# JiuTongBro/MultiView_Inpaint

Hardware: AMD Instinct MI355X
Metric: Mpix/s fwd+bwd @1.5M Gauss 1080p (higher is better)
Workload: dtype f32; 1 GPU; rasterizer-with-depth fwd+bwd, one 1920x1080 view per GPU per step, N=1500000 Gaussians, sh_degree 3 (BASELINE.json configs[2] size, SURVEY.md §8d scene); gaussians=1500000, visible=1312313, num_rendered_D=14779663, tiles=8160, tile_list_max=2266, parallelism=views x1

## Files before the change

include/mvi_raster.h:

```cpp
#ifndef MVI_RASTER_H
#define MVI_RASTER_H

#include <stddef.h>
#include <stdint.h>

#ifdef __cplusplus
extern "C" {
#endif

#define MVI_OK 0
#define MVI_EINVAL (-1)
#define MVI_EHIP (-2)
#define MVI_ENOMEM (-3)

#define MVI_TILE 16

typedef struct mvi_raster_settings {
    int32_t image_height;
    int32_t image_width;
    float tanfovx;
    float tanfovy;
    float scale_modifier;
    int32_t sh_degree;
    int32_t prefiltered;
// ... 65 lines not shown
                             const float* colors_precomp, const float* scales, const float* rotations,
                             const float* cov3D_precomp, const int32_t* radii, const void* geom,
                             const float* grad_rows_scratch, float* dL_dmeans3D, float* dL_dmeans2D, float* dL_dopacity,
                             float* dL_dshs, float* dL_dcolors, float* dL_dscales, float* dL_drotations, float* dL_dcov3D,
                             void* stream);

int mvi_raster_backward_geom_range(const mvi_raster_settings* s, int32_t P, int32_t M, int32_t first, int32_t count,
                                   const float* means3D, const float* shs, const float* colors_precomp, const float* scales,
                                   const float* rotations, const float* cov3D_precomp, const int32_t* radii, const void* geom,
                                   const float* grad_rows_scratch, float* dL_dmeans3D, float* dL_dmeans2D, float* dL_dopacity,
                                   float* dL_dshs, float* dL_dcolors, float* dL_dscales, float* dL_drotations, float* dL_dcov3D,
                                   void* stream);

typedef struct mvi_raster_views {
    const float* depths;
    const float* means2D;
    const float* cov3D_a;
    const float* cov3D_b;
    const float* conic_opacity;
    const float* rgbd;
    const uint32_t* tiles_touched;
    const uint8_t* clamped;
    const void* tile_ids_sorted;
    const uint32_t* point_list;
    const uint32_t* ranges;
    const float* final_T;
    const uint32_t* n_contrib;
    int32_t tile_id_bytes;
    const uint8_t* grad_support;
} mvi_raster_views;
int mvi_raster_get_views(int32_t P, int64_t num_rendered, int32_t image_width, int32_t image_height,
                         const void* geom, const void* binning, const void* image,
                         mvi_raster_views* out);

#define MVI_RASTER_NSTAGES 8
int mvi_raster_timing_enable(int enable);
int mvi_raster_timing_enable_stages(uint32_t stage_mask);
int mvi_raster_timing_read(float* ms_sum_host, int32_t* calls_host);
const char* mvi_raster_stage_name(int stage);

int mvi_raster_color_mode(int deferred);
int mvi_raster_resolve_colors(const mvi_raster_settings* s, int32_t P, void* geom, size_t geom_bytes, void* stream);

int mvi_raster_binning_version(int version);
int mvi_raster_backward_mode(int dense);
int mvi_raster_dev_stamps(int pass, void* device_buffer);
int mvi_raster_dev_wave_sum9(const float* in, float* out, int n_waves, void* stream);

const char* mvi_raster_last_error(void);
const char* mvi_version(void);

#ifdef __cplusplus
}
#endif
#endif
```

multiview_inpaint_amd/_lib.py:

```python
import ctypes as C
import os
import re

_HERE = os.path.dirname(os.path.abspath(__file__))
LIB_PATH = os.environ.get("MVI_HIP_LIB") or os.path.join(_HERE, "csrc", "libmvi_hip.so")
LIB_OVERRIDDEN = bool(os.environ.get("MVI_HIP_LIB"))
if LIB_OVERRIDDEN:
    import sys as _sys
    _sys.stderr.write(f"[mvi] MVI_HIP_LIB is set: every kernel comes from {LIB_PATH}, not from the in-tree build\n")
INCLUDE_DIR = os.path.normpath(os.path.join(_HERE, "..", "include"))


class RasterSettings(C.Structure):
    _fields_ = [
        ("image_height", C.c_int32), ("image_width", C.c_int32),
        ("tanfovx", C.c_float), ("tanfovy", C.c_float), ("scale_modifier", C.c_float),
        ("sh_degree", C.c_int32), ("prefiltered", C.c_int32),
        ("bg", C.c_void_p), ("viewmatrix", C.c_void_p), ("projmatrix", C.c_void_p), ("campos", C.c_void_p),
    ]


class RasterViews(C.Structure):
    _fields_ = [(n, C.c_void_p) for n in (
        "depths", "means2D", "cov3D_a", "cov3D_b", "conic_opacity", "rgbd", "tiles_touched", "clamped",
# ... 51 lines not shown
    L.mvi_version.restype = C.c_char_p
    L.mvi_raster_geom_bytes.restype = sz
    L.mvi_raster_geom_bytes.argtypes = [i32]
    L.mvi_raster_image_bytes.restype = sz
    L.mvi_raster_image_bytes.argtypes = [i32, i32]
    L.mvi_raster_binning_bytes.restype = sz
    L.mvi_raster_binning_bytes.argtypes = [i64, i32, i32]
    L.mvi_raster_forward_geom.restype = C.c_int
    L.mvi_raster_forward_geom.argtypes = [C.POINTER(RasterSettings), i32, i32] + [vp] * 7 + [vp, sz, vp, C.POINTER(i64), vp]
    L.mvi_raster_forward_render.restype = C.c_int
    L.mvi_raster_forward_render.argtypes = [C.POINTER(RasterSettings), i32, i64, vp, vp, sz, vp, sz, vp, sz, vp, vp, vp]
    L.mvi_raster_forward_render_prepare.restype = C.c_int
    L.mvi_raster_forward_render_prepare.argtypes = [C.POINTER(RasterSettings), i32, i64, vp, vp, sz, vp, sz, vp, sz, vp, vp, vp, vp]
    L.mvi_raster_backward.restype = C.c_int
    L.mvi_raster_backward.argtypes = [C.POINTER(RasterSettings), i32, i32, i64] + [vp] * 20 + [i32, vp]
    L.mvi_raster_backward_render.restype = C.c_int
    L.mvi_raster_backward_render.argtypes = [C.POINTER(RasterSettings), i32, i64] + [vp] * 7 + [i32, i32, vp]
    L.mvi_raster_backward_geom.restype = C.c_int
    L.mvi_raster_backward_geom.argtypes = [C.POINTER(RasterSettings), i32, i32] + [vp] * 18
    L.mvi_raster_backward_geom_range.restype = C.c_int
    L.mvi_raster_backward_geom_range.argtypes = [C.POINTER(RasterSettings), i32, i32, i32, i32] + [vp] * 18
    L.mvi_raster_forward_geom_raw.restype = C.c_int
    L.mvi_raster_forward_geom_raw.argtypes = [C.POINTER(RasterSettings), i32, i32] + [vp] * 6 + [vp, sz, vp, C.POINTER(i64), vp]
    L.mvi_raster_backward_raw.restype = C.c_int
    L.mvi_raster_backward_raw.argtypes = [C.POINTER(RasterSettings), i32, i32, i64] + [vp] * 19 + [i32, vp]
    L.mvi_raster_backward_raw_factor.restype = C.c_int
    L.mvi_raster_backward_raw_factor.argtypes = [C.POINTER(RasterSettings), i32, i32, i64] + [vp] * 18 + [i32, vp]
    L.mvi_raster_sh_backward_views.restype = C.c_int
    L.mvi_raster_sh_backward_views.argtypes = [i32, i32, i32, i32, vp, vp, i64, vp, i64, vp, vp]
    L.mvi_raster_mark_visible.restype = C.c_int
    L.mvi_raster_mark_visible.argtypes = [i32, vp, vp, vp, vp, vp]
    L.mvi_raster_get_views.restype = C.c_int
    L.mvi_raster_get_views.argtypes = [i32, i64, i32, i32, vp, vp, vp, C.POINTER(RasterViews)]
    L.mvi_raster_timing_enable.restype = C.c_int
    L.mvi_raster_timing_enable.argtypes = [C.c_int]
    L.mvi_raster_timing_enable_stages.restype = C.c_int
    L.mvi_raster_timing_enable_stages.argtypes = [C.c_uint32]
    L.mvi_raster_timing_read.restype = C.c_int
    L.mvi_raster_timing_read.argtypes = [C.POINTER(C.c_float), C.POINTER(C.c_int32)]
    L.mvi_raster_stage_name.restype = C.c_char_p
    L.mvi_raster_stage_name.argtypes = [C.c_int]
    L.mvi_raster_binning_version.restype = C.c_int
    L.mvi_raster_binning_version.argtypes = [C.c_int]
    L.mvi_raster_backward_mode.restype = C.c_int
    L.mvi_raster_backward_mode.argtypes = [C.c_int]
    L.mvi_raster_color_mode.restype = C.c_int
    L.mvi_raster_color_mode.argtypes = [C.c_int]
    L.mvi_raster_resolve_colors.restype = C.c_int
    L.mvi_raster_resolve_colors.argtypes = [C.POINTER(RasterSettings), i32, vp, sz, vp]
    L.mvi_raster_dev_stamps.restype = C.c_int
    L.mvi_raster_dev_stamps.argtypes = [C.c_int, vp]
    L.mvi_raster_dev_wave_sum9.restype = C.c_int
    L.mvi_raster_dev_wave_sum9.argtypes = [vp, vp, C.c_int, vp]
    _bind_unet_ops(L)
    _bind_train_ops(L)
    _bind_box_region(L)
    _lib = L
    return L


def _bind_unet_ops(L):
    try:
        from . import _unet_ops_bind
    except ImportError:
        return
    _unet_ops_bind.bind(L)
# ... 54 lines not shown
```

multiview_inpaint_amd/csrc/raster_api.hip:

```cpp
#include <cstdio>
#include <cstdlib>
#include <cstring>

#include "raster_common.h"

namespace mvi {
int launch_scan_block_sums(GeomView g, int P, unsigned long long* total_host_devptr, hipStream_t st);
int launch_zero_fill(void* p, size_t bytes, hipStream_t st);
int launch_binning_level1(const Frame& f, GeomView g, hipStream_t st);
}

static thread_local char g_err[512] = "";
static int g_dense_backward = [] { const char* e = getenv("MVI_RASTER_DENSE_BACKWARD"); return (e && e[0] == '1') ? 1 : 0; }();
static int g_defer_colors = [] { const char* e = getenv("MVI_RASTER_EAGER_COLORS"); return (e && e[0] == '1') ? 0 : 1; }();
#include <mutex>
namespace {
struct SegmentHint { const void* geom; int32_t P; int64_t segments; uint64_t stamp; };
constexpr int kSegmentHints = 64;
SegmentHint g_seg_hints[kSegmentHints] = {};
uint64_t g_seg_clock = 0;
std::mutex g_seg_mutex;
void remember_segments(const void* geom, int32_t P, int64_t segments) {
    std::lock_guard<std::mutex> lock(g_seg_mutex);
    int slot = 0;
// ... 495 lines not shown

int mvi_raster_mark_visible(int32_t P, const float* means3D, const float* viewmatrix, const float* projmatrix,
                            uint8_t* visible, void* stream) {
    if (P < 0 || (P > 0 && (!means3D || !viewmatrix || !visible))) return fail(MVI_EINVAL, "bad arguments to mark_visible%s");
    if (mvi::launch_mark_visible(P, means3D, viewmatrix, visible, (hipStream_t)stream)) return hip_fail("mark_visible", hipGetLastError());
    return MVI_OK;
}

int mvi_raster_get_views(int32_t P, int64_t D, int32_t W, int32_t H, const void* geom, const void* binning,
                         const void* image, mvi_raster_views* out) {
    if (!out) return fail(MVI_EINVAL, "views is NULL%s");
    memset(out, 0, sizeof(*out));
    if (geom) {
        mvi::GeomView g = mvi::carve_geom(const_cast<void*>(geom), P);
        out->depths = g.depths; out->means2D = reinterpret_cast<const float*>(g.xy);
        out->cov3D_a = reinterpret_cast<const float*>(g.cov_a); out->cov3D_b = reinterpret_cast<const float*>(g.cov_b);
        out->conic_opacity = reinterpret_cast<const float*>(g.conic_opacity); out->rgbd = reinterpret_cast<const float*>(g.rgbd);
        out->tiles_touched = g.tiles_touched; out->clamped = g.clamped;
        out->grad_support = g.touched;
    }
    if (binning) {
        mvi::BinningView b = mvi::carve_binning(const_cast<void*>(binning), D, W, H);
        int fin = b.passes & 1;
        out->tile_ids_sorted = b.keys[fin]; out->point_list = b.vals[fin];
        out->tile_id_bytes = b.key_bytes;
    }
    if (image) {
        mvi::ImageView im = mvi::carve_image(const_cast<void*>(image), W, H);
        out->ranges = im.ranges; out->final_T = im.final_T; out->n_contrib = im.n_contrib;
    }
    return MVI_OK;
}

}
```

multiview_inpaint_amd/csrc/raster_binning.hip:

```cpp
#include "raster_common.h"

namespace mvi {

__global__ __launch_bounds__(256) void zero_fill_kernel(uint4* __restrict__ p, size_t n16) {
    for (size_t i = (size_t)blockIdx.x * 256 + threadIdx.x; i < n16; i += (size_t)gridDim.x * 256) p[i] = make_uint4(0u, 0u, 0u, 0u);
}
int launch_zero_fill(void* p, size_t bytes, hipStream_t st) {
    if (bytes == 0) return 0;
    const size_t n16 = (bytes + 15) / 16;
    size_t blocks = (n16 + 255) / 256;
    if (blocks > 256 * 32) blocks = 256 * 32;
    hipLaunchKernelGGL(zero_fill_kernel, dim3((unsigned)blocks), dim3(256), 0, st, (uint4*)p, n16);
    return hipGetLastError() == hipSuccess ? 0 : MVI_EHIP;
}

__global__ __launch_bounds__(1024) void scan_block_sums_kernel(const uint32_t* __restrict__ sums,
                                                               uint32_t* __restrict__ offsets, int n) {
    __shared__ uint32_t s_wave[16];
    __shared__ uint32_t s_carry;
    const int tid = threadIdx.x, lane = tid & 63, wave = tid >> 6;
    if (tid == 0) s_carry = 0;
    __syncthreads();
    for (int base = 0; base < n; base += 1024) {
        int i = base + tid;
// ... 266 lines not shown
            s_val[lp] = val[it];
        }
    }
    __syncthreads();
    const int count = (int)((D - tile0) < kTileW ? (D - tile0) : kTileW);
#pragma unroll
    for (int it = 0; it < kSortItems; ++it) {
        int lp = it * kNT + tid;
        if (lp < count) {
            const KeyT kk = s_key[lp];
            uint32_t k = (uint32_t)kk;
            uint32_t d = (k >> shift) & mask;
            uint32_t dst = s_digit_base[d] + ((uint32_t)lp - s_local_start[d]);
            keys_out[dst] = kk;
            vals_out[dst] = s_val[lp];
        }
    }
}

template <typename KeyT>
__global__ __launch_bounds__(kBlock) void tile_ranges_kernel(const KeyT* __restrict__ tile_keys, int64_t D,
                                                             uint32_t* __restrict__ ranges) {
    int64_t i = (int64_t)blockIdx.x * kBlock + threadIdx.x;
    if (i >= D) return;
    uint32_t t = tile_keys[i];
    if (i == 0) ranges[2 * t] = 0;
    else {
        uint32_t tp = tile_keys[i - 1];
        if (t != tp) { ranges[2 * tp + 1] = (uint32_t)i; ranges[2 * t] = (uint32_t)i; }
    }
    if (i == D - 1) ranges[2 * t + 1] = (uint32_t)D;
}

__global__ __launch_bounds__(1024) void total_block_sums_kernel(const uint32_t* __restrict__ sums,
                                                                uint32_t* __restrict__ offsets, int n,
                                                                unsigned long long* __restrict__ total_host) {
    __shared__ unsigned long long s_wave[16];
    unsigned long long acc = 0;
    for (int i = threadIdx.x; i < n; i += 1024) acc += sums[i];
#pragma unroll
    for (int d = 32; d >= 1; d >>= 1) acc += __shfl_xor(acc, d);
    if ((threadIdx.x & 63) == 0) s_wave[threadIdx.x >> 6] = acc;
    __syncthreads();
    if (threadIdx.x == 0) {
        unsigned long long t = 0;
#pragma unroll
        for (int w = 0; w < 16; ++w) t += s_wave[w];
        offsets[n] = (uint32_t)t;
        if (total_host) __hip_atomic_store(total_host, t, __ATOMIC_RELEASE, __HIP_MEMORY_SCOPE_SYSTEM);
    }
}

int launch_scan_block_sums(GeomView g, int P, unsigned long long* total_host_devptr, hipStream_t st) {
    int nblk = (P + kPB - 1) / kPB;
    hipLaunchKernelGGL(total_block_sums_kernel, dim3(1), dim3(1024), 0, st, g.block_sums, g.block_offsets, nblk,
                       total_host_devptr);
    return hipGetLastError() == hipSuccess ? 0 : MVI_EHIP;
}

template <int kW, typename KeyT>
static int radix_pass(KeyT* const keys[2], uint32_t* const vals[2], int cur, int64_t n, int shift, int bits,
                      uint32_t* hist, uint32_t* tot, int nsort, hipStream_t st) {
    uint32_t mask = (1u << bits) - 1u;
    hipLaunchKernelGGL((radix_count_kernel<kW, KeyT>), dim3(nsort / kCountTiles), dim3(1024), 0, st, keys[cur], n, shift, mask, hist, nsort);
    hipLaunchKernelGGL(radix_scan_rows_kernel, dim3(256), dim3(1024), 0, st, hist, nsort, tot);
#define MVI_SCATTER(B)                                                                                                       \
// ... 67 lines not shown
```

multiview_inpaint_amd/csrc/raster_binning2.hip:

```cpp
#include <cstdlib>

#include "raster_common.h"

namespace mvi {

static int g_binning_version = [] { const char* e = getenv("MVI_BINNING_LEGACY"); return (e && e[0] == '1') ? 1 : 2; }();
bool binning_v2_enabled() { return g_binning_version == 2; }
int set_binning_version(int v) {
    const int old = g_binning_version;
    if (v == 1 || v == 2) g_binning_version = v;
    return old;
}

__device__ __forceinline__ uint32_t block_excl_scan256(uint32_t v, int tid, uint32_t* s_w4, uint32_t* total) {
    const int lane = tid & 63, wave = tid >> 6;
    uint32_t inc = v;
#pragma unroll
    for (int o = 1; o < 64; o <<= 1) {
        uint32_t t = __shfl_up(inc, o);
        if (lane >= o) inc += t;
    }
    if (wave < 4 && lane == 63) s_w4[wave] = inc;
    __syncthreads();
    uint32_t off = 0;
// ... 77 lines not shown
                }
            }
            atomicAdd(&s_h[d_prev], run);
        }
    }
    __syncthreads();
    const uint32_t c = s_h[tid];
    table[(size_t)blockIdx.x * 256 + tid] = c;
    if (c) atomicAdd(&super[(size_t)(blockIdx.x / kDsSuper) * 256 + tid], c);
}

template <int PASS>
__global__ __launch_bounds__(kDsThreads) void depth_scatter_kernel(
    const uint32_t* __restrict__ keys_in, const uint32_t* __restrict__ vals_in, uint32_t* __restrict__ keys_out,
    uint32_t* __restrict__ vals_out, int P, const uint32_t* __restrict__ table, const uint32_t* __restrict__ super,
    int nsuper, uint32_t* __restrict__ super_next, const uint2* __restrict__ rect, uint2* __restrict__ rect_sorted) {
    constexpr int kW = kDsThreads / 64;
    constexpr int shift = 8 * PASS;
    __shared__ uint32_t s_wave_hist[kW][256];
    __shared__ unsigned long long s_match[kW][256];
    __shared__ uint32_t s_digit_base[256];
    __shared__ uint32_t s_local_start[256];
    __shared__ uint32_t s_red[4][2][256];
    __shared__ uint32_t s_w4[4];
    __shared__ uint32_t s_key[kDsTile];
    __shared__ uint32_t s_val[kDsTile];
    const int tid = threadIdx.x, lane = tid & 63, wave = tid >> 6;
#pragma unroll
    for (int i = tid; i < kW * 256; i += kDsThreads) { (&s_wave_hist[0][0])[i] = 0; (&s_match[0][0])[i] = 0ull; }

    const int tile0 = blockIdx.x * kDsTile;
    const int base = tile0 + wave * (kDsItems * 64);
    uint32_t key[kDsItems], val[kDsItems];
#pragma unroll
    for (int it = 0; it < kDsItems; ++it) {
        const int idx = base + it * 64 + lane;
        const bool valid = idx < P;
        key[it] = valid ? keys_in[idx] : 0u;
        val[it] = PASS == 0 ? (uint32_t)idx : (valid ? vals_in[idx] : 0u);
    }
    uint2 rc[PASS == 3 ? kDsItems : 1];
    if (PASS == 3) {
#pragma unroll
        for (int it = 0; it < kDsItems; ++it)
            rc[it] = (base + it * 64 + lane) < P ? rect[val[it]] : make_uint2(0u, 0u);
    }
    {
        const int dq = tid & 63, rg = tid >> 6;
        const int grp = (int)blockIdx.x / kDsSuper;
        uint4 all = make_uint4(0u, 0u, 0u, 0u), bef = make_uint4(0u, 0u, 0u, 0u);
#pragma unroll 4
        for (int j = rg; j < nsuper; j += 4) {
            const uint4 c = *reinterpret_cast<const uint4*>(super + (size_t)j * 256 + 4 * dq);
            all.x += c.x; all.y += c.y; all.z += c.z; all.w += c.w;
            if (j < grp) { bef.x += c.x; bef.y += c.y; bef.z += c.z; bef.w += c.w; }
        }
#pragma unroll
        for (int j = rg; j < kDsSuper - 1; j += 4) {
            const int t = grp * kDsSuper + j;
            if (t < (int)blockIdx.x) {
                const uint4 c = *reinterpret_cast<const uint4*>(table + (size_t)t * 256 + 4 * dq);
                bef.x += c.x; bef.y += c.y; bef.z += c.z; bef.w += c.w;
            }
        }
        *reinterpret_cast<uint4*>(&s_red[rg][0][4 * dq]) = all;
        *reinterpret_cast<uint4*>(&s_red[rg][1][4 * dq]) = bef;
        if (super_next && blockIdx.x == 0)
            for (int i = tid; i < 256 * nsuper; i += kDsThreads) super_next[i] = 0u;
    }
    __syncthreads();
    const uint32_t all = s_red[0][0][tid] + s_red[1][0][tid] + s_red[2][0][tid] + s_red[3][0][tid];
    const uint32_t before = s_red[0][1][tid] + s_red[1][1][tid] + s_red[2][1][tid] + s_red[3][1][tid];
    uint32_t dinc = all;
#pragma unroll
    for (int o = 1; o < 64; o <<= 1) {
        uint32_t t = __shfl_up(dinc, o);
        if (lane >= o) dinc += t;
    }
// ... 54 lines not shown
            const uint32_t d = dig[it];
            const uint32_t lp = s_local_start[d] + s_wave_hist[wave][d] + rank[it];
            s_key[lp] = key[it];
            s_val[lp] = val[it];
            if (PASS == 3) rect_sorted[s_digit_base[d] + (lp - s_local_start[d])] = rc[it];
        }
    }
    __syncthreads();
    const int count = (P - tile0) < kDsTile ? (P - tile0) : kDsTile;
#pragma unroll
    for (int it = 0; it < kDsItems; ++it) {
        const int lp = it * kDsThreads + tid;
        if (lp < count) {
            const uint32_t k = s_key[lp];
            const uint32_t d = (k >> shift) & 255u;
            const uint32_t dst = s_digit_base[d] + ((uint32_t)lp - s_local_start[d]);
            if (PASS != 3) keys_out[dst] = k;
            vals_out[dst] = s_val[lp];
        }
    }
}

__global__ __launch_bounds__(kExThreads) void column_count_kernel(int P, int gx, const uint2* __restrict__ rect_sorted,
                                                                  uint32_t* __restrict__ col_table, int nblk1) {
    __shared__ uint32_t s_d[257];
    __shared__ uint32_t s_w4[4];
    const int tid = threadIdx.x;
    if (tid <= 256) s_d[tid] = 0;
    const int base = blockIdx.x * kExChunk;
    uint2 rc[kExItems];
#pragma unroll
    for (int k = 0; k < kExItems; ++k) {
        const int i = base + k * kExThreads + tid;
        rc[k] = i < P ? rect_sorted[i] : make_uint2(0u, 0u);
    }
    __syncthreads();
#pragma unroll
    for (int k = 0; k < kExItems; ++k) {
        const uint32_t x0 = rc[k].x & 0xFFFFu, w = rc[k].y & 0xFFFFu, h = rc[k].y >> 16;
        if (w * h) { atomicAdd(&s_d[x0], 1u); atomicSub(&s_d[x0 + w], 1u); }
    }
    __syncthreads();
    const uint32_t v = tid < 256 ? s_d[tid] : 0u;
    const uint32_t ex = block_excl_scan256(v, tid, s_w4, nullptr);
    if (tid < gx) col_table[(size_t)tid * nblk1 + blockIdx.x] = ex + v;
}

__device__ __forceinline__ void build_chunk_table(const uint32_t* col_tot, int gx, int tid, uint32_t* __restrict__ chunk_first,
                                                  uint32_t* __restrict__ col_start, uint32_t* s_w4) {
    const uint32_t v = tid < gx ? __hip_atomic_load(col_tot + tid, __ATOMIC_RELAXED, __HIP_MEMORY_SCOPE_AGENT) : 0u;
    const uint32_t c = tid < gx ? max(1u, (v + (uint32_t)kEx2Chunk - 1u) / (uint32_t)kEx2Chunk) : 0u;
    uint32_t tv, tc;
    const uint32_t ev = block_excl_scan256(v, tid, s_w4, &tv);
    const uint32_t ec = block_excl_scan256(c, tid, s_w4, &tc);
    if (tid < gx) { col_start[tid] = ev; chunk_first[tid] = ec; }
    if (tid == 0) { col_start[gx] = tv; chunk_first[gx] = tc; }
}
__global__ __launch_bounds__(1024) void columns_scan_kernel(uint32_t* __restrict__ table, int stride, int n,
                                                            uint32_t* __restrict__ tot, int gx, uint32_t* __restrict__ arrivals,
                                                            uint32_t* __restrict__ chunk_first,
                                                            uint32_t* __restrict__ col_start) {
    __shared__ uint32_t s_wave[16];
    __shared__ uint32_t s_carry, s_last;
    __shared__ uint32_t s_w4[4];
    uint32_t* row = table + (size_t)blockIdx.x * stride;
    const int tid = threadIdx.x, lane = tid & 63, wave = tid >> 6;
    if (tid == 0) s_carry = 0;
    __syncthreads();
// ... 26 lines not shown
    __syncthreads();
    if (!s_last) return;
    build_chunk_table(tot, gx, tid, chunk_first, col_start, s_w4);
}
struct Chunk { int x; uint32_t seg0, seg1; bool first; };
__device__ __forceinline__ bool load_chunk(const uint32_t* __restrict__ chunk_first, const uint32_t* __restrict__ col_start,
                                           int gx, int tid, uint32_t* s_first, uint32_t* s_col, Chunk& ck) {
    if (tid <= gx) { s_first[tid] = chunk_first[tid]; s_col[tid] = col_start[tid]; }
    __syncthreads();
    const uint32_t c = blockIdx.x;
    if (c >= s_first[gx]) return false;
    int lo = 0, hi = gx - 1;
    while (lo < hi) {
        const int mid = (lo + hi + 1) >> 1;
        if (s_first[mid] <= c) lo = mid; else hi = mid - 1;
    }
    ck.x = lo;
    ck.first = c == s_first[lo];
    ck.seg0 = s_col[lo] + (c - s_first[lo]) * (uint32_t)kEx2Chunk;
    ck.seg1 = min(ck.seg0 + (uint32_t)kEx2Chunk, s_col[lo + 1]);
    return true;
}

__global__ __launch_bounds__(kExThreads) void row_count_kernel(int gx, int gy, const uint32_t* __restrict__ chunk_first,
                                                               const uint32_t* __restrict__ col_start,
                                                               const uint16_t* __restrict__ seg_yh,
                                                               uint32_t* __restrict__ row_table, int stride) {
    __shared__ uint32_t s_first[257], s_col[257], s_w4[4];
    __shared__ uint32_t s_d[257];
    const int tid = threadIdx.x;
    if (tid <= 256) s_d[tid] = 0;
    Chunk ck;
    if (!load_chunk(chunk_first, col_start, gx, tid, s_first, s_col, ck)) return;
#pragma unroll
    for (int k = 0; k < kEx2Items; ++k) {
        const uint32_t i = ck.seg0 + (uint32_t)(k * kExThreads + tid);
        if (i < ck.seg1) {
            const uint32_t yh = seg_yh[i];
            const uint32_t y0 = yh & 255u, h = (yh >> 8) + 1u;
            atomicAdd(&s_d[y0], 1u);
            atomicSub(&s_d[y0 + h], 1u);
        }
    }
    __syncthreads();
    const uint32_t v = tid < 256 ? s_d[tid] : 0u;
    const uint32_t ex = block_excl_scan256(v, tid, s_w4, nullptr);
    if (tid < gy) row_table[(size_t)tid * stride + blockIdx.x] = ex + v;
}

__global__ __launch_bounds__(1024) void row_scan_kernel(int gx, const uint32_t* __restrict__ chunk_first,
                                                        uint32_t* __restrict__ row_table, int stride,
                                                        uint32_t* __restrict__ row_tot, uint32_t* __restrict__ col_rel) {
    __shared__ uint32_t s_first[257];
    __shared__ uint32_t s_wave[16];
    __shared__ uint32_t s_carry;
    const int tid = threadIdx.x, lane = tid & 63, wave = tid >> 6;
    if (tid <= gx) s_first[tid] = chunk_first[tid];
    if (tid == 0) s_carry = 0;
    __syncthreads();
    const int n = (int)s_first[gx];
    uint32_t* row = row_table + (size_t)blockIdx.x * stride;
    for (int base = 0; base < n; base += 1024) {
        const int i = base + tid;
        const uint32_t v = i < n ? row[i] : 0u;
        uint32_t inc = v;
#pragma unroll
        for (int o = 1; o < 64; o <<= 1) {
            uint32_t t = __shfl_up(inc, o);
            if (lane >= o) inc += t;
        }
        if (lane == 63) s_wave[wave] = inc;
// ... 57 lines not shown
}

template <int PASS, int NB, int ITEMS, int CAP>
__global__ __launch_bounds__(kExThreads) void expand_scatter_kernel(ExpandArgs A) {
    constexpr int kChunk = kExThreads * ITEMS;
    constexpr int kCap = CAP;
    constexpr int kRounds = kChunk / 64;
    constexpr int kStride = NB + 1;
    static_assert(kCap >= 64 * NB, "a round of 64 items (<= 64 * NB entries) always fits the image");
    static_assert(kRounds >= 16, "worker parts <= rounds");
    static_assert(kExThreads == 512, "block_excl_scan512x2");
    __shared__ alignas(16) unsigned long long s_mask[kRounds * kStride + 1];
    __shared__ uint32_t s_pay[kChunk];
    __shared__ uint16_t s_aux[PASS == 1 ? kChunk : 1];
    __shared__ uint32_t s_img[kCap];
    __shared__ uint32_t s_lstart[NB + 1], s_delta[NB];
    __shared__ uint32_t s_rtot[kRounds];
    __shared__ uint32_t s_w[2][8];
    uint32_t* const s_first = s_img;
    uint32_t* const s_col = s_img + 257;
    const int tid = threadIdx.x, lane = tid & 63, wave = tid >> 6;
    const uint32_t blk = blockIdx.x;

    uint32_t item0 = 0, item1 = 0;
    Chunk ck{0, 0u, 0u, false};
    if (PASS == 1) {
        item0 = blk * (uint32_t)kChunk;
        item1 = min(item0 + (uint32_t)kChunk, (uint32_t)A.n_items);
    } else {
        if (!load_chunk(A.chunk_first, A.col_start, A.gx, tid, s_first, s_col, ck)) return;
        item0 = ck.seg0; item1 = ck.seg1;
    }
    MVI_STAMP(0);
    uint32_t ia[ITEMS], in_[ITEMS];
#pragma unroll
    for (int k = 0; k < ITEMS; ++k) {
        const int li = (wave * ITEMS + k) * 64 + lane;
        const uint32_t i = item0 + (uint32_t)li;
        ia[k] = 0; in_[k] = 0;
        uint32_t pay = 0, aux = 0;
        if (i < item1) {
            if (PASS == 1) {
                const uint2 rc = A.rect_sorted[i];
                const uint32_t w = rc.y & 0xFFFFu, h = rc.y >> 16;
                if (w * h) {
                    ia[k] = rc.x & 0xFFFFu; in_[k] = w;
                    pay = A.order[i];
                    aux = (rc.x >> 16) | ((h - 1u) << 8);
                }
            } else {
                const uint32_t yh = A.seg_yh_in[i];
                ia[k] = yh & 255u; in_[k] = (yh >> 8) + 1u;
                pay = A.seg_idx_in[i];
            }
        }
        s_pay[li] = pay;
        if (PASS == 1) s_aux[li] = (uint16_t)aux;
    }
    const int nb = A.nbins;
    const int parts = min(kExThreads / nb, 16);
    const bool worker = tid < parts * nb;
    const int b = worker ? tid / parts : 0, q = worker ? tid % parts : 0;
    const int r_lo = worker ? q * kRounds / parts : 0, r_hi = worker ? (q + 1) * kRounds / parts : 0;
    const bool bin_head = worker && q == 0;
    const uint32_t bin_tot = bin_head ? A.tot[b] : 0u;
    const uint32_t bin_off = bin_head ? A.table[(size_t)b * A.stride + blk] : 0u;
    {
        uint4* m4 = reinterpret_cast<uint4*>(&s_mask[0]);
        for (int i = tid; i < (kRounds * kStride + 1) / 2; i += kExThreads) m4[i] = make_uint4(0u, 0u, 0u, 0u);
        if (tid < kRounds) s_rtot[tid] = 0;
    }
    __syncthreads();
    MVI_STAMP(1);

    const unsigned long long bit = 1ull << lane;
#pragma unroll
    for (int k = 0; k < ITEMS; ++k) {
        unsigned long long* row = s_mask + (wave * ITEMS + k) * kStride;
        for (uint32_t i = 0; i < in_[k]; ++i) atomicOr(&row[ia[k] + i], bit);
    }
    __syncthreads();
    MVI_STAMP(2);

    const unsigned long long* mcol = s_mask + b;
    uint32_t my_base = 0, my_goff = 0;

    int g0 = 0, g1 = kRounds;
    bool first = true, have_rtot = false;
    for (;;) {
        uint32_t cnt = 0;
        for (int r = max(r_lo, g0); r < min(r_hi, g1); ++r) cnt += (uint32_t)__popcll(mcol[r * kStride]);
        uint32_t pos0, total, bin_start;
        block_excl_scan512x2(cnt, first ? bin_tot : 0u, tid, s_w, pos0, total, bin_start);
        if (first) {
            first = false;
            my_base = bin_start + bin_off;
            if (PASS == 2 && ck.first && bin_head) {
                const uint32_t* cr = A.col_rel + (size_t)b * (A.gx + 1);
                const uint32_t c = cr[ck.x + 1] - cr[ck.x];
                uint2* rg = reinterpret_cast<uint2*>(A.ranges) + ((size_t)b * A.gx + ck.x);
                *rg = c ? make_uint2(my_base, my_base + c) : make_uint2(0u, 0u);
            }
            if (total == 0) return;
// ... 16 lines not shown
        if (bin_head) {
            s_lstart[b] = pos0;
            s_delta[b] = my_base + my_goff - pos0;
        }
        if (tid == 0) s_lstart[nb] = total;
        MVI_STAMP(4);
        if (cnt) {
            uint32_t pos = pos0;
            const uint32_t hi = (uint32_t)b << 16;
            for (int r = max(r_lo, g0); r < min(r_hi, g1); ++r) {
                const unsigned long long m = mcol[r * kStride];
                uint32_t m0 = (uint32_t)m, m1 = (uint32_t)(m >> 32);
                const uint32_t item_hi = hi | (uint32_t)(r * 64);
                while (m0) {
                    const uint32_t l = (uint32_t)__builtin_ctz(m0);
                    m0 &= m0 - 1u;
                    s_img[pos++] = item_hi | l;
                }
                while (m1) {
                    const uint32_t l = (uint32_t)__builtin_ctz(m1);
                    m1 &= m1 - 1u;
                    s_img[pos++] = item_hi | 32u | l;
                }
            }
        }
        __syncthreads();
        MVI_STAMP(5);
        for (uint32_t p = tid; p < total; p += kExThreads) {
            const uint32_t e = s_img[p];
            const uint32_t eb = e >> 16, item = e & 0xFFFFu;
            const uint32_t dst = p + s_delta[eb];
            A.out_idx[dst] = s_pay[item];
            if (PASS == 1) A.out_aux[dst] = s_aux[item];
            else A.out_aux[dst] = (uint16_t)(eb * (uint32_t)A.gx + (uint32_t)ck.x);
        }
        MVI_STAMP(6);
        if (g1 >= kRounds) break;
        if (bin_head) my_goff += s_lstart[b + 1] - pos0;
        __syncthreads();
        g0 = g1; g1 = kRounds;
    }
}

int launch_binning2_level1(const Frame& f, GeomView g, hipStream_t st) {
    if (f.P <= 0) return 0;
    {
        StageTimer tm(kStSort, st);
#define MVI_DS_PASS(PASS, SRC, DST)                                                                                              \
        hipLaunchKernelGGL(depth_count_kernel, dim3(g.nds), dim3(kDsThreads), 0, st, g.dkeys[SRC], f.P, 8 * PASS, g.ds_table,     \
                           g.ds_super[PASS & 1]);                                                                                 \
        hipLaunchKernelGGL((depth_scatter_kernel<PASS>), dim3(g.nds), dim3(kDsThreads), 0, st, g.dkeys[SRC], g.dvals[SRC],        \
                           g.dkeys[DST], g.dvals[DST], f.P, g.ds_table, g.ds_super[PASS & 1], g.nsuper,                           \
                           PASS < 3 ? g.ds_super[(PASS + 1) & 1] : (uint32_t*)nullptr, g.rect, g.rect_sorted);
        MVI_DS_PASS(0, 0, 1) MVI_DS_PASS(1, 1, 0) MVI_DS_PASS(2, 0, 1) MVI_DS_PASS(3, 1, 0)
#undef MVI_DS_PASS
    }
    StageTimer tm(kStDup, st);
    hipLaunchKernelGGL(column_count_kernel, dim3(g.nblk1), dim3(kExThreads), 0, st, f.P, f.gx, g.rect_sorted, g.col_table,
                       g.nblk1);
    hipLaunchKernelGGL(columns_scan_kernel, dim3(f.gx), dim3(1024), 0, st, g.col_table, g.nblk1, g.nblk1, g.col_tot, f.gx,
                       g.arrivals, g.chunk_first, g.col_start);
    return hipGetLastError() == hipSuccess ? 0 : MVI_EHIP;
}

int launch_binning2(const Frame& f, GeomView g, BinningView b, ImageView im, int64_t D, int64_t segments, hipStream_t st) {
    const size_t tiles = (size_t)f.gx * f.gy;
    if (D <= 0 || f.P <= 0) return launch_zero_fill(im.ranges, 8 * tiles, st);
    const bool wide = f.gx > 128 || f.gy > 128;
    ExpandArgs a1{};
    a1.n_items = f.P; a1.nbins = f.gx; a1.gx = f.gx;
    a1.order = g.dvals[0]; a1.rect_sorted = g.rect_sorted;
    a1.table = g.col_table; a1.tot = g.col_tot; a1.stride = g.nblk1;
    a1.out_idx = b.vals[0]; a1.out_aux = (uint16_t*)b.keys[0];
    a1.stamps = g_dev_stamps[0];
    {
        StageTimer tm(kStDup, st);
        if (wide)
            hipLaunchKernelGGL((expand_scatter_kernel<1, 256, kExItems, 64 * 256>), dim3(g.nblk1), dim3(kExThreads), 0, st, a1);
        else hipLaunchKernelGGL((expand_scatter_kernel<1, 128, kExItems, 64 * 128>), dim3(g.nblk1), dim3(kExThreads), 0, st, a1);
    }
    int nchunk = b.nsort;
    if (segments > 0 && segments <= D) nchunk = (int)min((int64_t)b.nsort, segments / kEx2Chunk + f.gx + 1);
    ExpandArgs a2{};
    a2.nbins = f.gy; a2.gx = f.gx;
    a2.chunk_first = g.chunk_first; a2.col_start = g.col_start;
    a2.seg_idx_in = b.vals[0]; a2.seg_yh_in = (const uint16_t*)b.keys[0];
    a2.col_rel = b.col_rel; a2.ranges = im.ranges;
    a2.table = b.block_hist; a2.tot = b.digit_tot; a2.stride = b.nsort;
    a2.out_idx = b.vals[1]; a2.out_aux = (uint16_t*)b.keys[1];
    a2.stamps = g_dev_stamps[1];
    StageTimer tm(kStSort, st);
    hipLaunchKernelGGL(row_count_kernel, dim3(nchunk), dim3(kExThreads), 0, st, f.gx, f.gy, g.chunk_first, g.col_start,
                       (const uint16_t*)b.keys[0], b.block_hist, b.nsort);
    hipLaunchKernelGGL(row_scan_kernel, dim3(f.gy), dim3(1024), 0, st, f.gx, g.chunk_first, b.block_hist, b.nsort,
                       b.digit_tot, b.col_rel);
    if (f.gy <= kEx2SmallNB)
        hipLaunchKernelGGL((expand_scatter_kernel<2, kEx2SmallNB, kEx2Items, kEx2SmallCap>), dim3(nchunk), dim3(kExThreads), 0,
                           st, a2);
    else if (f.gy <= 128)
        hipLaunchKernelGGL((expand_scatter_kernel<2, 128, kEx2Items, 64 * 128>), dim3(nchunk), dim3(kExThreads), 0, st, a2);
    else hipLaunchKernelGGL((expand_scatter_kernel<2, 256, kEx2Items, 64 * 256>), dim3(nchunk), dim3(kExThreads), 0, st, a2);
    return hipGetLastError() == hipSuccess ? 0 : MVI_EHIP;
}

}
```

multiview_inpaint_amd/csrc/raster_common.h:

```cpp
#pragma once
#include <hip/hip_runtime.h>
#include <stdint.h>
#include <stddef.h>
#include <type_traits>

#include "../../include/mvi_raster.h"

namespace mvi {

constexpr int kTile = MVI_TILE;
constexpr int kBlock = 256;
constexpr int kPB = 64;
constexpr float kNearZ = 0.2f;
constexpr float kLowpass = 0.3f;
constexpr float kFrustumClamp = 1.3f;
constexpr float kLambdaFloor = 0.1f;
constexpr float kAlphaMax = 0.99f;
constexpr float kAlphaMin = 1.0f / 255.0f;
constexpr float kTEps = 0.0001f;
constexpr float kDepthSentinel = 15.0f;

constexpr int kSortItems = 8;
constexpr int kSortWavesP = 4;
constexpr int kSortWavesD = 8;
// ... 443 lines not shown
        const uint32_t per = (z.n_body[r] + gridDim.x - 1) / gridDim.x;
        const size_t z0 = (size_t)blockIdx.x * per;
        typedef uint32_t zero_u32x4 __attribute__((ext_vector_type(4)));
        const zero_u32x4 zz = {0u, 0u, 0u, 0u};
        for (uint32_t i = tid; i < per && z0 + i < z.n_body[r]; i += nthreads)
            asm volatile("global_store_dwordx4 %0, %1, off sc1" ::"v"(z.body[r] + z0 + i), "v"(zz) : "memory");
        if (blockIdx.x == 0) {
            if (tid < (int)z.n_head[r]) z.head[r][tid] = 0.f;
            if (tid < (int)z.n_tail[r]) z.tail[r][tid] = 0.f;
        }
    }
}
int launch_zero_regions(const ZeroRegions& z, hipStream_t st);

int launch_preprocess_forward(const Frame& f, const float* means3D, const float* shs,
                              const float* colors_precomp, const float* opacities, const float* scales,
                              const float* rotations, const float* cov3D_precomp, GeomView g,
                              int32_t* radii, hipStream_t st);
struct RawBackwardExtra { const float* raw_opacity = nullptr; float* dL_dshs_rest = nullptr; int rows_prezeroed = 0; };
int launch_preprocess_backward_sparse(const Frame& f, const float* means3D, const float* shs, const float* scales,
                                      const float* rotations, const float* cov3D_precomp, GeomView g, const float* grad_rows,
                                      float* dL_dmeans3D, float* dL_dmeans2D, float* dL_dopacity, float* dL_dcolors,
                                      float* dL_dshs, float* dL_dcov3D, float* dL_dscales, float* dL_drots, hipStream_t st,
                                      RawBackwardExtra raw);
int launch_preprocess_backward(const Frame& f, const float* means3D, const float* shs,
                               const float* scales, const float* rotations, const float* cov3D_precomp,
                               const int32_t* radii, GeomView g, const float* grad_rows, float* dL_dmeans3D,
                               float* dL_dmeans2D, float* dL_dopacity, float* dL_dcolors, float* dL_dshs,
                               float* dL_dcov3D, float* dL_dscales, float* dL_drots, hipStream_t st,
                               RawBackwardExtra raw = RawBackwardExtra());
int launch_binning(const Frame& f, GeomView g, const int32_t* radii, BinningView b, ImageView im,
                   int64_t D, hipStream_t st);
int launch_zero_fill(void* p, size_t bytes, hipStream_t st);
int launch_binning2_totals(GeomView g, int P, unsigned long long* totals_host_devptr, hipStream_t st);
int launch_binning2_level1(const Frame& f, GeomView g, hipStream_t st);
int launch_binning2(const Frame& f, GeomView g, BinningView b, ImageView im, int64_t D, int64_t segments, hipStream_t st);
int launch_render_forward(const Frame& f, GeomView g, BinningView b, ImageView im, int64_t D,
                          float* out_color, float* out_depth, hipStream_t st, float* zero_rows = nullptr);
int launch_resolve_colors(const Frame& f, GeomView g, hipStream_t st);
int launch_render_backward(const Frame& f, GeomView g, BinningView b, ImageView im, int64_t D,
                           const float* dL_dpix, float* grad_rows, hipStream_t st, const ZeroRegions* zero = nullptr);
int launch_wave_sum9_probe(const float* in, float* out, int n_waves, hipStream_t st);
constexpr int kGradRow = 16;
int launch_sh_backward_views(int P, int M, int deg, int n_views, const float* means3D, const float* campos,
                             int64_t campos_stride, const float* gcol, int64_t gcol_stride, float* dL_dshs, hipStream_t st);
int launch_mark_visible(int P, const float* means3D, const float* view, uint8_t* visible, hipStream_t st);
int launch_color_factors(int P, const int32_t* radii, const float* grad_rows, const uint8_t* clamped, float* out, hipStream_t st);

}
```

multiview_inpaint_amd/raster/__init__.py:

```python
import ctypes as C
from typing import NamedTuple, Optional

import torch

from .. import _lib


class GaussianRasterizationSettings(NamedTuple):
    image_height: int
    image_width: int
    tanfovx: float
    tanfovy: float
    bg: torch.Tensor
    scale_modifier: float
    viewmatrix: torch.Tensor
    projmatrix: torch.Tensor
    sh_degree: int
    campos: torch.Tensor
    prefiltered: bool


def _ptr(t: Optional[torch.Tensor]):
    return None if t is None or t.numel() == 0 else C.c_void_p(t.data_ptr())

# ... 14 lines not shown
        s = _lib.RasterSettings()
        s.image_height, s.image_width = int(rs.image_height), int(rs.image_width)
        s.tanfovx, s.tanfovy, s.scale_modifier = float(rs.tanfovx), float(rs.tanfovy), float(rs.scale_modifier)
        s.sh_degree, s.prefiltered = int(rs.sh_degree), int(bool(rs.prefiltered))
        s.bg, s.viewmatrix, s.projmatrix, s.campos = (t.data_ptr() for t in self.keep)
        self.c = s


class RasterState:
    __slots__ = ("P", "M", "D", "W", "H", "geom", "binning", "image", "radii", "grad_rows", "rows_clean", "frame", "sources")

    def resolve_colors(self):
        if self.P == 0:
            return
        dev = self.geom.device
        stream = C.c_void_p(torch.cuda.current_stream(dev).cuda_stream)
        with torch.cuda.device(dev):
            _lib.check(_lib.lib().mvi_raster_resolve_colors(C.byref(self.frame.c), self.P, _ptr(self.geom), self.geom.numel(), stream),
                       "resolve_colors")

    def take_rows(self, dev):
        if getattr(self, "grad_rows", None) is not None and getattr(self, "rows_clean", False):
            self.rows_clean = False
            return self.grad_rows, 1
        return torch.empty(self.P, 16, dtype=torch.float32, device=dev), 0

    def views(self):
        L = _lib.lib()
        v = _lib.RasterViews()
        _lib.check(L.mvi_raster_get_views(self.P, self.D, self.W, self.H, _ptr(self.geom), _ptr(self.binning),
                                          _ptr(self.image), C.byref(v)), "get_views")
        return v

    def tensor(self, name, shape, dtype):
        v = self.views()
        addr = getattr(v, name)
        n = 1
        for s in shape:
            n *= s
        if name == "tile_ids_sorted" and v.tile_id_bytes == 2 and torch.empty(0, dtype=dtype).element_size() == 4:
            raw = self.tensor(name, tuple(shape) + (2,), torch.uint8).to(torch.int32)
            return (raw[..., 0] | (raw[..., 1] << 8)).to(dtype)
        out = torch.empty(shape, dtype=dtype, device=self.geom.device)
        if n:
            nbytes = n * out.element_size()
            for buf in (self.geom, self.binning, self.image):
                if buf is not None and buf.numel() and buf.data_ptr() <= addr < buf.data_ptr() + buf.numel():
                    off = addr - buf.data_ptr()
                    out.view(torch.uint8).reshape(-1).copy_(buf[off:off + nbytes])
                    return out
            raise RuntimeError(f"view {name} not inside a scratch buffer")
        return out


def _forward_render(L, fr, st, color, depth, stream, prepare_backward, dev):
    st.grad_rows, st.rows_clean = None, False
    if prepare_backward and st.P > 0:
        st.grad_rows = torch.empty(st.P, 16, dtype=torch.float32, device=dev)
        _lib.check(L.mvi_raster_forward_render_prepare(C.byref(fr.c), st.P, st.D, _ptr(st.radii), _ptr(st.geom), st.geom.numel(),
                                                       _ptr(st.binning), st.binning.numel(), _ptr(st.image), st.image.numel(),
                                                       _ptr(color), _ptr(depth), _ptr(st.grad_rows), stream),
                   "rasterize forward (render)")
        st.rows_clean = True
        return
    _lib.check(L.mvi_raster_forward_render(C.byref(fr.c), st.P, st.D, _ptr(st.radii), _ptr(st.geom), st.geom.numel(),
                                           _ptr(st.binning), st.binning.numel(), _ptr(st.image), st.image.numel(),
                                           _ptr(color), _ptr(depth), stream), "rasterize forward (render)")


def rasterize_forward(rs: GaussianRasterizationSettings, means3D, opacities, shs=None, colors_precomp=None,
                      scales=None, rotations=None, cov3D_precomp=None, prepare_backward=False):
    L = _lib.lib()
    fr = _Frame(rs)
    dev = means3D.device
# ... 329 lines not shown
```

Before: 2289 Mpix/s.

## Drop per-entry tile-id writes in binning sort and derive them lazily from ranges

The second binning pass no longer writes a 16-bit tile id per rendered entry into the aux key buffer. A new kernel rebuilds those ids from the per-tile ranges, and it runs only when the Python tensor view asks for tile_ids_sorted. Several binning kernels also clamp their indices so global loads can be issued early and without branches, then mask the results afterwards to overlap load latency. This removes roughly D×2 bytes of scattered stores from the timed step, at the cost of extra redundant loads at the tail and a lazy path that depends on the debug accessor.

```diff
diff --git a/include/mvi_raster.h b/include/mvi_raster.h
--- a/include/mvi_raster.h
+++ b/include/mvi_raster.h
@@ -121,6 +121,8 @@
 int mvi_raster_get_views(int32_t P, int64_t num_rendered, int32_t image_width, int32_t image_height,
                          const void* geom, const void* binning, const void* image,
                          mvi_raster_views* out);
+int mvi_raster_materialize_tile_ids(int32_t P, int64_t num_rendered, int32_t image_width, int32_t image_height,
+                                    void* binning, const void* image, void* stream);
 
 #define MVI_RASTER_NSTAGES 8
 int mvi_raster_timing_enable(int enable);
diff --git a/multiview_inpaint_amd/_lib.py b/multiview_inpaint_amd/_lib.py
--- a/multiview_inpaint_amd/_lib.py
+++ b/multiview_inpaint_amd/_lib.py
@@ -107,6 +107,8 @@
     L.mvi_raster_mark_visible.argtypes = [i32, vp, vp, vp, vp, vp]
     L.mvi_raster_get_views.restype = C.c_int
     L.mvi_raster_get_views.argtypes = [i32, i64, i32, i32, vp, vp, vp, C.POINTER(RasterViews)]
+    L.mvi_raster_materialize_tile_ids.restype = C.c_int
+    L.mvi_raster_materialize_tile_ids.argtypes = [i32, i64, i32, i32, vp, vp, vp]
     L.mvi_raster_timing_enable.restype = C.c_int
     L.mvi_raster_timing_enable.argtypes = [C.c_int]
     L.mvi_raster_timing_enable_stages.restype = C.c_int
diff --git a/multiview_inpaint_amd/csrc/raster_api.hip b/multiview_inpaint_amd/csrc/raster_api.hip
--- a/multiview_inpaint_amd/csrc/raster_api.hip
+++ b/multiview_inpaint_amd/csrc/raster_api.hip
@@ -551,4 +551,15 @@
     return MVI_OK;
 }
 
-}
+int mvi_raster_materialize_tile_ids(int32_t P, int64_t D, int32_t W, int32_t H, void* binning, const void* image, void* stream) {
+    if (P < 0 || D < 0 || W < 0 || H < 0) return fail(MVI_EINVAL, "negative size in materialize_tile_ids%s");
+    if (P == 0 || D == 0) return MVI_OK;
+    if (!binning || !image) return fail(MVI_EINVAL, "NULL scratch in materialize_tile_ids%s");
+    const int tiles = ((W + mvi::kTile - 1) / mvi::kTile) * ((H + mvi::kTile - 1) / mvi::kTile);
+    mvi::BinningView b = mvi::carve_binning(binning, D, W, H);
+    mvi::ImageView im = mvi::carve_image(const_cast<void*>(image), W, H);
+    if (mvi::launch_tile_ids_from_ranges(tiles, b, im, D, (hipStream_t)stream)) return hip_fail("materialize_tile_ids", hipGetLastError());
+    return MVI_OK;
+}
+
+}
diff --git a/multiview_inpaint_amd/csrc/raster_binning.hip b/multiview_inpaint_amd/csrc/raster_binning.hip
--- a/multiview_inpaint_amd/csrc/raster_binning.hip
+++ b/multiview_inpaint_amd/csrc/raster_binning.hip
@@ -322,6 +322,23 @@
     if (i == D - 1) ranges[2 * t + 1] = (uint32_t)D;
 }
 
+template <typename KeyT>
+__global__ __launch_bounds__(kBlock) void tile_ids_from_ranges_kernel(const uint2* __restrict__ ranges, int64_t D,
+                                                                      KeyT* __restrict__ tile_keys) {
+    const uint2 r = ranges[blockIdx.x];
+    const int64_t r1 = (int64_t)r.y < D ? (int64_t)r.y : D;
+    for (int64_t i = (int64_t)r.x + threadIdx.x; i < r1; i += kBlock) tile_keys[i] = (KeyT)blockIdx.x;
+}
+int launch_tile_ids_from_ranges(int tiles, BinningView b, ImageView im, int64_t D, hipStream_t st) {
+    if (tiles <= 0 || D <= 0) return 0;
+    void* keys = b.keys[b.passes & 1];
+    const uint2* ranges = reinterpret_cast<const uint2*>(im.ranges);
+    if (b.key_bytes == 2)
+        hipLaunchKernelGGL((tile_ids_from_ranges_kernel<uint16_t>), dim3(tiles), dim3(kBlock), 0, st, ranges, D, (uint16_t*)keys);
+    else hipLaunchKernelGGL((tile_ids_from_ranges_kernel<uint32_t>), dim3(tiles), dim3(kBlock), 0, st, ranges, D, (uint32_t*)keys);
+    return hipGetLastError() == hipSuccess ? 0 : MVI_EHIP;
+}
+
 __global__ __launch_bounds__(1024) void total_block_sums_kernel(const uint32_t* __restrict__ sums,
                                                                 uint32_t* __restrict__ offsets, int n,
                                                                 unsigned long long* __restrict__ total_host) {
diff --git a/multiview_inpaint_amd/csrc/raster_binning2.hip b/multiview_inpaint_amd/csrc/raster_binning2.hip
--- a/multiview_inpaint_amd/csrc/raster_binning2.hip
+++ b/multiview_inpaint_amd/csrc/raster_binning2.hip
@@ -133,18 +133,28 @@
     const int tile0 = blockIdx.x * kDsTile;
     const int base = tile0 + wave * (kDsItems * 64);
     uint32_t key[kDsItems], val[kDsItems];
-#pragma unroll
-    for (int it = 0; it < kDsItems; ++it) {
-        const int idx = base + it * 64 + lane;
-        const bool valid = idx < P;
-        key[it] = valid ? keys_in[idx] : 0u;
-        val[it] = PASS == 0 ? (uint32_t)idx : (valid ? vals_in[idx] : 0u);
-    }
     uint2 rc[PASS == 3 ? kDsItems : 1];
     if (PASS == 3) {
 #pragma unroll
-        for (int it = 0; it < kDsItems; ++it)
-            rc[it] = (base + it * 64 + lane) < P ? rect[val[it]] : make_uint2(0u, 0u);
+        for (int it = 0; it < kDsItems; ++it) val[it] = vals_in[min(base + it * 64 + lane, P - 1)];
+#pragma unroll
+        for (int it = 0; it < kDsItems; ++it) key[it] = keys_in[min(base + it * 64 + lane, P - 1)];
+#pragma unroll
+        for (int it = 0; it < kDsItems; ++it) {
+            const bool valid = (base + it * 64 + lane) < P;
+            key[it] = valid ? key[it] : 0u;
+            val[it] = valid ? val[it] : 0u;
+        }
+#pragma unroll
+        for (int it = 0; it < kDsItems; ++it) rc[it] = rect[val[it]];
+    } else {
+#pragma unroll
+        for (int it = 0; it < kDsItems; ++it) {
+            const int idx = base + it * 64 + lane;
+            const bool valid = idx < P;
+            key[it] = valid ? keys_in[idx] : 0u;
+            val[it] = PASS == 0 ? (uint32_t)idx : (valid ? vals_in[idx] : 0u);
+        }
     }
     {
         const int dq = tid & 63, rg = tid >> 6;
@@ -265,8 +275,11 @@
 #pragma unroll
     for (int k = 0; k < kExItems; ++k) {
         const int i = base + k * kExThreads + tid;
-        rc[k] = i < P ? rect_sorted[i] : make_uint2(0u, 0u);
-    }
+        rc[k] = rect_sorted[min(i, P - 1)];
+    }
+#pragma unroll
+    for (int k = 0; k < kExItems; ++k)
+        if (base + k * kExThreads + tid >= P) rc[k] = make_uint2(0u, 0u);
     __syncthreads();
 #pragma unroll
     for (int k = 0; k < kExItems; ++k) {
@@ -359,11 +372,15 @@
     if (tid <= 256) s_d[tid] = 0;
     Chunk ck;
     if (!load_chunk(chunk_first, col_start, gx, tid, s_first, s_col, ck)) return;
+    const uint32_t last = ck.seg1 ? ck.seg1 - 1u : 0u;
+    uint32_t yhs[kEx2Items];
+#pragma unroll
+    for (int k = 0; k < kEx2Items; ++k) yhs[k] = seg_yh[min(ck.seg0 + (uint32_t)(k * kExThreads + tid), last)];
 #pragma unroll
     for (int k = 0; k < kEx2Items; ++k) {
         const uint32_t i = ck.seg0 + (uint32_t)(k * kExThreads + tid);
         if (i < ck.seg1) {
-            const uint32_t yh = seg_yh[i];
+            const uint32_t yh = yhs[k];
             const uint32_t y0 = yh & 255u, h = (yh >> 8) + 1u;
             atomicAdd(&s_d[y0], 1u);
             atomicSub(&s_d[y0 + h], 1u);
@@ -487,30 +504,14 @@
         item0 = ck.seg0; item1 = ck.seg1;
     }
     MVI_STAMP(0);
-    uint32_t ia[ITEMS], in_[ITEMS];
+    const uint32_t last = PASS == 1 ? (uint32_t)A.n_items - 1u : (item1 ? item1 - 1u : 0u);
+    uint2 ld_rc[PASS == 1 ? ITEMS : 1];
+    uint32_t ld_pay[ITEMS], ld_yh[PASS == 2 ? ITEMS : 1];
 #pragma unroll
     for (int k = 0; k < ITEMS; ++k) {
-        const int li = (wave * ITEMS + k) * 64 + lane;
-        const uint32_t i = item0 + (uint32_t)li;
-        ia[k] = 0; in_[k] = 0;
-        uint32_t pay = 0, aux = 0;
-        if (i < item1) {
-            if (PASS == 1) {
-                const uint2 rc = A.rect_sorted[i];
-                const uint32_t w = rc.y & 0xFFFFu, h = rc.y >> 16;
-                if (w * h) {
-                    ia[k] = rc.x & 0xFFFFu; in_[k] = w;
-                    pay = A.order[i];
-                    aux = (rc.x >> 16) | ((h - 1u) << 8);
-                }
-            } else {
-                const uint32_t yh = A.seg_yh_in[i];
-                ia[k] = yh & 255u; in_[k] = (yh >> 8) + 1u;
-                pay = A.seg_idx_in[i];
-            }
-        }
-        s_pay[li] = pay;
-        if (PASS == 1) s_aux[li] = (uint16_t)aux;
+        const uint32_t i = min(item0 + (uint32_t)((wave * ITEMS + k) * 64 + lane), last);
+        if (PASS == 1) { ld_rc[k] = A.rect_sorted[i]; ld_pay[k] = A.order[i]; }
+        else { ld_yh[k] = A.seg_yh_in[i]; ld_pay[k] = A.seg_idx_in[i]; }
     }
     const int nb = A.nbins;
     const int parts = min(kExThreads / nb, 16);
@@ -524,6 +525,26 @@
         uint4* m4 = reinterpret_cast<uint4*>(&s_mask[0]);
         for (int i = tid; i < (kRounds * kStride + 1) / 2; i += kExThreads) m4[i] = make_uint4(0u, 0u, 0u, 0u);
         if (tid < kRounds) s_rtot[tid] = 0;
+    }
+    uint32_t ia[ITEMS], in_[ITEMS];
+#pragma unroll
+    for (int k = 0; k < ITEMS; ++k) {
+        const int li = (wave * ITEMS + k) * 64 + lane;
+        const bool inside = item0 + (uint32_t)li < item1;
+        if (PASS == 1) {
+            const uint2 rc = ld_rc[k];
+            const uint32_t w = rc.y & 0xFFFFu, h = rc.y >> 16;
+            const bool on = inside && w * h != 0u;
+            ia[k] = on ? rc.x & 0xFFFFu : 0u;
+            in_[k] = on ? w : 0u;
+            s_pay[li] = on ? ld_pay[k] : 0u;
+            s_aux[li] = on ? (uint16_t)((rc.x >> 16) | ((h - 1u) << 8)) : (uint16_t)0;
+        } else {
+            const uint32_t yh = ld_yh[k];
+            ia[k] = inside ? yh & 255u : 0u;
+            in_[k] = inside ? (yh >> 8) + 1u : 0u;
+            s_pay[li] = inside ? ld_pay[k] : 0u;
+        }
     }
     __syncthreads();
     MVI_STAMP(1);
@@ -606,7 +627,6 @@
             const uint32_t dst = p + s_delta[eb];
             A.out_idx[dst] = s_pay[item];
             if (PASS == 1) A.out_aux[dst] = s_aux[item];
-            else A.out_aux[dst] = (uint16_t)(eb * (uint32_t)A.gx + (uint32_t)ck.x);
         }
         MVI_STAMP(6);
         if (g1 >= kRounds) break;
@@ -661,7 +681,7 @@
     a2.seg_idx_in = b.vals[0]; a2.seg_yh_in = (const uint16_t*)b.keys[0];
     a2.col_rel = b.col_rel; a2.ranges = im.ranges;
     a2.table = b.block_hist; a2.tot = b.digit_tot; a2.stride = b.nsort;
-    a2.out_idx = b.vals[1]; a2.out_aux = (uint16_t*)b.keys[1];
+    a2.out_idx = b.vals[1];
     a2.stamps = g_dev_stamps[1];
     StageTimer tm(kStSort, st);
     hipLaunchKernelGGL(row_count_kernel, dim3(nchunk), dim3(kExThreads), 0, st, f.gx, f.gy, g.chunk_first, g.col_start,
diff --git a/multiview_inpaint_amd/csrc/raster_common.h b/multiview_inpaint_amd/csrc/raster_common.h
--- a/multiview_inpaint_amd/csrc/raster_common.h
+++ b/multiview_inpaint_amd/csrc/raster_common.h
@@ -499,6 +499,7 @@
 int launch_binning(const Frame& f, GeomView g, const int32_t* radii, BinningView b, ImageView im,
                    int64_t D, hipStream_t st);
 int launch_zero_fill(void* p, size_t bytes, hipStream_t st);
+int launch_tile_ids_from_ranges(int tiles, BinningView b, ImageView im, int64_t D, hipStream_t st);
 int launch_binning2_totals(GeomView g, int P, unsigned long long* totals_host_devptr, hipStream_t st);
 int launch_binning2_level1(const Frame& f, GeomView g, hipStream_t st);
 int launch_binning2(const Frame& f, GeomView g, BinningView b, ImageView im, int64_t D, int64_t segments, hipStream_t st);
diff --git a/multiview_inpaint_amd/raster/__init__.py b/multiview_inpaint_amd/raster/__init__.py
--- a/multiview_inpaint_amd/raster/__init__.py
+++ b/multiview_inpaint_amd/raster/__init__.py
@@ -70,14 +70,20 @@
                                           _ptr(self.image), C.byref(v)), "get_views")
         return v
 
-    def tensor(self, name, shape, dtype):
+    def tensor(self, name, shape, dtype, _derive=True):
         v = self.views()
         addr = getattr(v, name)
+        if _derive and name == "tile_ids_sorted" and self.D > 0 and self.binning is not None and self.image is not None:
+            dev = self.binning.device
+            with torch.cuda.device(dev):
+                _lib.check(_lib.lib().mvi_raster_materialize_tile_ids(
+                    self.P, self.D, self.W, self.H, _ptr(self.binning), _ptr(self.image),
+                    C.c_void_p(torch.cuda.current_stream(dev).cuda_stream)), "materialize_tile_ids")
         n = 1
         for s in shape:
             n *= s
         if name == "tile_ids_sorted" and v.tile_id_bytes == 2 and torch.empty(0, dtype=dtype).element_size() == 4:
-            raw = self.tensor(name, tuple(shape) + (2,), torch.uint8).to(torch.int32)
+            raw = self.tensor(name, tuple(shape) + (2,), torch.uint8, _derive=False).to(torch.int32)
             return (raw[..., 0] | (raw[..., 1] << 8)).to(dtype)
         out = torch.empty(shape, dtype=dtype, device=self.geom.device)
         if n:
```

New measurement: 2317 Mpix/s, median of 6. 1.2% higher.
